# ShuhangGu/DASR

Measured on AMD Instinct MI355X. Metric: SR train images/sec (4x, 128->512), higher is better.
Workload: dtype bf16 MFMA operands, fp32 accumulate / fp32 residual stream

## Files before the change

dasr_amd/csrc/common.h:

```cpp
#pragma once
#include <hip/hip_runtime.h>
#include <hip/hip_ext.h>
#include <stdint.h>
#include "../../include/dasr_hip.h"

typedef __bf16 bf16_t;
typedef __attribute__((ext_vector_type(8))) __bf16 bf16x8;
typedef __attribute__((ext_vector_type(4))) __bf16 bf16x4;
typedef __attribute__((ext_vector_type(4))) short s16x4;
typedef _Float16 f16_t;
typedef __attribute__((ext_vector_type(8))) _Float16 f16x8;
typedef __attribute__((ext_vector_type(4))) _Float16 f16x4;
typedef __attribute__((ext_vector_type(16))) float f32x16;
typedef __attribute__((ext_vector_type(4))) float f32x4;
typedef __attribute__((ext_vector_type(4))) unsigned int u32x4;
typedef __attribute__((ext_vector_type(2))) unsigned int u32x2;

#define DASR_LDS __attribute__((address_space(3)))

#define HIP_TRY(expr)                                   \
    do {                                                \
        hipError_t _e = (expr);                         \
        if (_e != hipSuccess) return (int)_e;           \
    } while (0)

__device__ __forceinline__ float bf16_to_f32(bf16_t v) { return (float)v; }

__device__ __forceinline__ bf16_t f32_to_bf16(float v) { return (bf16_t)v; }

__device__ __forceinline__ void split_bf16(float v, bf16_t& hi, bf16_t& lo) {
    hi = (bf16_t)v;
    lo = (bf16_t)(v - (float)hi);
}

__device__ __forceinline__ void split_f16(float v, bf16_t& hi, bf16_t& lo) {
    const f16_t h = (f16_t)v;
    hi = __builtin_bit_cast(bf16_t, h);
    lo = __builtin_bit_cast(bf16_t, (f16_t)(v - (float)h));
}

template <bool F16>
__device__ __forceinline__ f32x16 mfma16(bf16x8 a, bf16x8 b, f32x16 c) {
    if constexpr (F16) return __builtin_amdgcn_mfma_f32_32x32x16_f16(__builtin_bit_cast(f16x8, a), __builtin_bit_cast(f16x8, b), c, 0, 0, 0);
    else return __builtin_amdgcn_mfma_f32_32x32x16_bf16(a, b, c, 0, 0, 0);
}

__device__ __forceinline__ float wave_sum(float v) {
#pragma unroll
    for (int o = 32; o > 0; o >>= 1) v += __shfl_xor(v, o, 64);
    return v;
}

static inline hipStream_t as_stream(void* s) { return (hipStream_t)s; }

struct dasr_red {
    float* part;
    unsigned* ticket;
};
dasr_red dasr_red_scratch(const void* key_acc, hipStream_t s, unsigned nblocks, int k);
int dasr_red_error();

template <int K>
__device__ __forceinline__ void grid_sum_commit(const dasr_red r, const float (&v)[K], float* const (&acc)[K], const float (&coef)[K]) {
    if (!r.part) return;
    __shared__ unsigned gs_last;
    __shared__ float gs_red[K][4];
    const unsigned nb = gridDim.x;
    if (threadIdx.x == 0) {
#pragma unroll
        for (int k = 0; k < K; ++k) __hip_atomic_store(r.part + (size_t)k * nb + blockIdx.x, v[k], __ATOMIC_RELAXED, __HIP_MEMORY_SCOPE_AGENT);
        asm volatile("s_waitcnt vmcnt(0)" ::: "memory");
        gs_last = __hip_atomic_fetch_add(r.ticket, 1u, __ATOMIC_RELAXED, __HIP_MEMORY_SCOPE_AGENT) == nb - 1u;
    }
    __syncthreads();
    if (!gs_last) return;
#pragma unroll
    for (int k = 0; k < K; ++k) {
        float s = 0.f;
        for (unsigned i = threadIdx.x; i < nb; i += 256u) s += __hip_atomic_load(r.part + (size_t)k * nb + i, __ATOMIC_RELAXED, __HIP_MEMORY_SCOPE_AGENT);
        s = wave_sum(s);
        if ((threadIdx.x & 63) == 0) gs_red[k][threadIdx.x >> 6] = s;
    }
    __syncthreads();
    if (threadIdx.x == 0) {
#pragma unroll
        for (int k = 0; k < K; ++k)
            if (acc[k]) atomicAdd(acc[k], ((gs_red[k][0] + gs_red[k][1]) + (gs_red[k][2] + gs_red[k][3])) * coef[k]);
        __hip_atomic_store(r.ticket, 0u, __ATOMIC_RELAXED, __HIP_MEMORY_SCOPE_AGENT);
    }
}

bool dasr_prof_slot(const char* tag, hipEvent_t* e0, hipEvent_t* e1);
#define DASR_LAUNCH_TAG(tag, kfn, grid, block, lds, s, ...)                                         \
    do {                                                                                            \
        hipEvent_t _e0 = nullptr, _e1 = nullptr;                                                    \
        if (dasr_prof_slot(tag, &_e0, &_e1)) hipExtLaunchKernelGGL(kfn, grid, block, lds, s, _e0, _e1, 0, __VA_ARGS__); \
        else hipLaunchKernelGGL(kfn, grid, block, lds, s, __VA_ARGS__);                             \
    } while (0)
#define DASR_LAUNCH(kfn, ...) DASR_LAUNCH_TAG(#kfn, kfn, __VA_ARGS__)
```

dasr_amd/csrc/misc.hip:

```cpp
#include "common.h"
#include <string.h>
#include <atomic>
#include <condition_variable>
#include <map>
#include <mutex>
#include <thread>
#include <tuple>

namespace {

__global__ void pack_kernel(const dasr_pack_desc* __restrict__ descs, int ndesc, long long total,
                            const long long* __restrict__ prefix, const float* __restrict__ params, bf16_t* __restrict__ packed) {
    const long long gid = (long long)blockIdx.x * blockDim.x + threadIdx.x;
    if (gid >= total) return;
    int lo = 0, hi = ndesc - 1;
    while (lo < hi) {
        const int mid = (lo + hi + 1) >> 1;
        if (prefix[mid] <= gid) lo = mid; else hi = mid - 1;
    }
    const dasr_pack_desc& D = descs[lo];
    long long q = gid - prefix[lo];
    const int lane = q & 63;
    q >>= 6;
    const int mi = q % D.mt;
    q /= D.mt;
    const int tap = q % D.ntaps;
    q /= D.ntaps;
    const int nchunks = D.cin_pad >> 4;
    const int ckv = q % nchunks;
    const int mg = q / nchunks;
    const int oc = (mg * D.mt + mi) * 32 + (lane & 31);
    const int kreal = D.fmt >= 3 ? nchunks / 3 : nchunks;
    const int part = ckv / kreal, ck = ckv - part * kreal;
    const int c0 = ck * 16 + 8 * (lane >> 5);
    bf16x8 vh, vl;
#pragma unroll
    for (int e = 0; e < 8; ++e) {
        const int cin = c0 + e;
        float v = 0.f;
        if (oc < D.cout) {
            for (int s = 0; s < D.nseg; ++s) {
                const dasr_pack_seg& S = D.seg[s];
                const int ci = cin - S.cin_start;
                if (ci >= 0 && ci < S.cin_len) {
                    const int st = D.tapmap[tap];
                    const unsigned msk = tap < 16 ? D.tapmask[tap] : 0u;
                    const bool okc = !S.transpose || ci < S.src_cout;
                    const long long base = !S.transpose ? S.src_off + ((long long)oc * S.src_cin + S.src_c0 + ci) * D.src_ntaps
                                                        : S.src_off + ((long long)ci * S.src_cin + S.src_c0 + oc) * D.src_ntaps;
                    if (msk && okc) {
                        float acc = 0.f;
                        for (int k = 0; k < D.src_ntaps && k < 16; ++k)
                            if (msk & (1u << k)) acc += params[base + k];
                        v = acc;
                    } else if (st >= 0 && okc) {
                        v = params[base + st];
                    }
                }
            }
        }
        bf16_t h, l;
        split_bf16(v, h, l);
        if (D.fmt == 1) h = __builtin_bit_cast(bf16_t, (f16_t)v);
        if (D.fmt == 2 || D.fmt == 3) split_f16(v, h, l);
        if (D.fmt >= 3 && part == 2) h = l;
        vh[e] = h;
        vl[e] = l;
    }
    const long long o = D.dst_off + (gid - prefix[lo]) * 8;
    *(bf16x8*)(packed + o) = vh;
    if (D.lo_off) *(bf16x8*)(packed + o + D.lo_off) = vl;
}

__global__ void nchw_to_blocked_kernel(const float* __restrict__ src, int N, int C, int H, int W, dasr_tensor df, dasr_tensor db) {
    const int ncb = (C + 15) >> 4;
    const long long total = (long long)N * ncb * H * W;
    const long long i = (long long)blockIdx.x * blockDim.x + threadIdx.x;
    if (i >= total) return;
    const int x = i % W;
    long long t = i / W;
    const int y = t % H;
    t /= H;
    const int cb = t % ncb;
    const int n = t / ncb;
    float v[16];
#pragma unroll
    for (int j = 0; j < 16; ++j) {
        const int c = cb * 16 + j;
        v[j] = c < C ? src[(((long long)n * C + c) * H + y) * W + x] : 0.f;
    }
    const size_t po = ((size_t)y * W + x) * 16;
    if (df.p) {
        float* d = (float*)df.p + (size_t)n * df.n_stride + (size_t)cb * df.cb_stride + po;
#pragma unroll
        for (int j = 0; j < 4; ++j) ((f32x4*)d)[j] = f32x4{v[4 * j], v[4 * j + 1], v[4 * j + 2], v[4 * j + 3]};
    }
    if (db.p) {
        bf16_t* d = (bf16_t*)db.p + (size_t)n * db.n_stride + (size_t)cb * db.cb_stride + po;
        bf16x8 a, b;
#pragma unroll
        for (int j = 0; j < 8; ++j) {
            a[j] = (bf16_t)v[j];
            b[j] = (bf16_t)v[8 + j];
        }
        ((bf16x8*)d)[0] = a;
        ((bf16x8*)d)[1] = b;
    }
}

__global__ void blocked_to_nchw_kernel(dasr_tensor s, int N, int C, int H, int W, float* __restrict__ dst) {
    const long long total = (long long)N * C * H * W;
    const long long i = (long long)blockIdx.x * blockDim.x + threadIdx.x;
    if (i >= total) return;
    const int x = i % W;
    long long t = i / W;
    const int y = t % H;
    t /= H;
    const int c = t % C;
    const int n = t / C;
    dst[i] = ((const float*)s.p)[(size_t)n * s.n_stride + (size_t)(c >> 4) * s.cb_stride + ((size_t)y * W + x) * 16 + (c & 15)];
}

__global__ void l1_loss_kernel(dasr_tensor sr, const float* __restrict__ hr, const float* __restrict__ wm, int N, int C, int H, int W,
                               float coef, float* loss_acc, dasr_tensor grad, int accumulate, float gscale, dasr_red rs) {
    const long long total = (long long)N * H * W;
    const long long i = (long long)blockIdx.x * blockDim.x + threadIdx.x;
    float part = 0.f;
    if (i < total) {
        const int x = i % W;
        long long t = i / W;
        const int y = t % H;
        const int n = t / H;
        const size_t po = ((size_t)y * W + x) * 16;
        const float* s = (const float*)sr.p + (size_t)n * sr.n_stride + po;
        const float wgt = wm ? wm[((long long)n * H + y) * W + x] : 1.f;
        float g[16];
#pragma unroll
        for (int j = 0; j < 16; ++j) g[j] = 0.f;
        for (int c = 0; c < C; ++c) {
            const float d = s[c] - hr[(((long long)n * C + c) * H + y) * W + x];
            if (accumulate & 2) {
                part += wgt * d * d;
                g[c] = 2.f * coef * wgt * d;
            } else {
                part += wgt * fabsf(d);
                g[c] = coef * wgt * (d > 0.f ? 1.f : (d < 0.f ? -1.f : 0.f));
            }
        }
        if (grad.p && (accumulate & 4)) {
            f16_t* gp = (f16_t*)grad.p + (size_t)n * grad.n_stride + po;
            for (int j = 0; j < (C + 3) / 4; ++j) {
                f16x4 o;
#pragma unroll
                for (int e = 0; e < 4; ++e) o[e] = (f16_t)(g[4 * j + e] * gscale);
                ((f16x4*)gp)[j] = o;
            }
        } else if (grad.p) {
            float* gp = (float*)grad.p + (size_t)n * grad.n_stride + po;
#pragma unroll
            for (int j = 0; j < 4; ++j) {
                f32x4 o = {g[4 * j], g[4 * j + 1], g[4 * j + 2], g[4 * j + 3]};
                if (accumulate & 1) o += ((const f32x4*)gp)[j];
                ((f32x4*)gp)[j] = o;
            }
        }
    }
    part = wave_sum(part);
    __shared__ float red[4];
    if ((threadIdx.x & 63) == 0) red[threadIdx.x >> 6] = part;
    __syncthreads();
    const float v[1] = {red[0] + red[1] + red[2] + red[3]};
    float* const acc[1] = {loss_acc};
    const float cf[1] = {coef};
    grid_sum_commit<1>(rs, v, acc, cf);
}

__global__ void downsum2x_kernel(dasr_tensor src, int N, int C, int H, int W, dasr_tensor mask, int mask_f32, float slope,
                                 dasr_tensor df, dasr_tensor db) {
    const int ncb = (C + 15) >> 4;
    const long long total = (long long)N * ncb * H * W * 4;
    const long long gi = (long long)blockIdx.x * blockDim.x + threadIdx.x;
    if (gi >= total) return;
    const int q = gi & 3;
    const long long i = gi >> 2;
    const int x = i % W;
    long long t = i / W;
    const int y = t % H;
    t /= H;
    const int cb = t % ncb;
    const int n = t / ncb;
    const float* s = (const float*)src.p + (size_t)n * src.n_stride + (size_t)cb * src.cb_stride + q * 4;
    const int W2 = 2 * W;
    f32x4 a = *(const f32x4*)(s + ((size_t)(2 * y) * W2 + 2 * x) * 16);
    a += *(const f32x4*)(s + ((size_t)(2 * y) * W2 + 2 * x + 1) * 16);
    a += *(const f32x4*)(s + ((size_t)(2 * y + 1) * W2 + 2 * x) * 16);
    a += *(const f32x4*)(s + ((size_t)(2 * y + 1) * W2 + 2 * x + 1) * 16);
    const size_t po = ((size_t)y * W + x) * 16 + q * 4;
    if (mask.p) {
        const size_t mo = (size_t)n * mask.n_stride + (size_t)cb * mask.cb_stride + po;
        float m[4];
        if (mask_f32) {
            const f32x4 mv = *(const f32x4*)((const float*)mask.p + mo);
            for (int j = 0; j < 4; ++j) m[j] = mv[j];
        } else {
            const bf16x4 mv = *(const bf16x4*)((const bf16_t*)mask.p + mo);
            for (int j = 0; j < 4; ++j) m[j] = (float)mv[j];
        }
        for (int j = 0; j < 4; ++j) a[j] = m[j] > 0.f ? a[j] : a[j] * slope;
    }
    if (df.p) *(f32x4*)((float*)df.p + (size_t)n * df.n_stride + (size_t)cb * df.cb_stride + po) = a;
    if (db.p) {
        bf16x4 o;
        for (int j = 0; j < 4; ++j) o[j] = (bf16_t)a[j];
        *(bf16x4*)((bf16_t*)db.p + (size_t)n * db.n_stride + (size_t)cb * db.cb_stride + po) = o;
    }
}

__global__ void axpby_kernel(dasr_tensor x, float a, dasr_tensor z, float b, int N, int C, int H, int W, dasr_tensor of,
                             dasr_tensor ob, float gamma, dasr_tensor mask, float slope, const float* slope_ptr) {
    const int ncb = (C + 15) >> 4;
    const long long per_plane = (long long)H * W * 4;
    const long long total = (long long)N * ncb * per_plane;
    const long long gi = (long long)blockIdx.x * blockDim.x + threadIdx.x;
    if (gi >= total) return;
    const long long e = (gi % per_plane) * 4;
    long long t = gi / per_plane;
    const int cb = t % ncb;
    const int n = t / ncb;
    f32x4 v = *(const f32x4*)((const float*)x.p + (size_t)n * x.n_stride + (size_t)cb * x.cb_stride + e) * a;
    if (z.p) v += *(const f32x4*)((const float*)z.p + (size_t)n * z.n_stride + (size_t)cb * z.cb_stride + e) * b;
    if (mask.p) {
        const float sl = slope_ptr ? *slope_ptr : slope;
        const f32x4 mv = *(const f32x4*)((const float*)mask.p + (size_t)n * mask.n_stride + (size_t)cb * mask.cb_stride + e);
        for (int j = 0; j < 4; ++j) v[j] = mv[j] > 0.f ? v[j] : v[j] * sl;
    }
    if (of.p) *(f32x4*)((float*)of.p + (size_t)n * of.n_stride + (size_t)cb * of.cb_stride + e) = v;
    if (ob.p) {
        bf16x4 o;
        for (int j = 0; j < 4; ++j) o[j] = (bf16_t)(v[j] * gamma);
        *(bf16x4*)((bf16_t*)ob.p + (size_t)n * ob.n_stride + (size_t)cb * ob.cb_stride + e) = o;
    }
}

__global__ void adam_kernel(float* __restrict__ p, const float* __restrict__ g, float* __restrict__ m, float* __restrict__ v,
                            long long n, float step_size, float beta1, float beta2, float eps, float wd, float inv_sqrt_bc2, int* __restrict__ nonfinite,
                            const int* __restrict__ gate) {
    if (gate && *gate != 0) return;
    bool bad = false;
    for (long long i = (long long)blockIdx.x * blockDim.x + threadIdx.x; i < n; i += (long long)gridDim.x * blockDim.x) {
        float gi = g[i];
        bad |= !(fabsf(gi) <= 3.0e38f);
        const float pi = p[i];
        if (wd != 0.f) gi += wd * pi;
        const float mi = beta1 * m[i] + (1.f - beta1) * gi;
        const float vi = beta2 * v[i] + (1.f - beta2) * gi * gi;
        m[i] = mi;
        v[i] = vi;
        const float denom = sqrtf(vi) * inv_sqrt_bc2 + eps;
        p[i] = pi - step_size * (mi / denom);
    }
    if (nonfinite && __any(bad) && (threadIdx.x & 63) == 0) atomicOr(nonfinite, 1);
}

__global__ void add_flat_kernel(float* __restrict__ y, const float* __restrict__ x, long long n) {
    for (long long i = (long long)blockIdx.x * blockDim.x + threadIdx.x; i < n; i += (long long)gridDim.x * blockDim.x) y[i] += x[i];
}

__global__ void fill_kernel(float* p, long long n, float v) {
    for (long long i = (long long)blockIdx.x * blockDim.x + threadIdx.x; i < n; i += (long long)gridDim.x * blockDim.x) p[i] = v;
}

inline unsigned blocks_for(long long total, int bs = 256) { return (unsigned)((total + bs - 1) / bs); }

}

extern "C" int dasr_pack_weights(const dasr_pack_desc* descs_dev, int32_t ndesc, int64_t total_pieces, const int64_t* piece_prefix_dev,
                                 const float* params_flat, void* packed, void* stream) {
    if (ndesc <= 0 || total_pieces <= 0) return DASR_EINVAL;
    DASR_LAUNCH(pack_kernel, dim3(blocks_for(total_pieces)), dim3(256), 0, as_stream(stream), descs_dev, ndesc,
                       (long long)total_pieces, (const long long*)piece_prefix_dev, params_flat, (bf16_t*)packed);
    return (int)hipGetLastError();
}

extern "C" int dasr_nchw_to_blocked(const float* src, int32_t N, int32_t C, int32_t H, int32_t W, dasr_tensor dst_f32,
                                    dasr_tensor dst_bf16, void* stream) {
    const long long total = (long long)N * ((C + 15) / 16) * H * W;
    if (total <= 0) return DASR_EINVAL;
    DASR_LAUNCH(nchw_to_blocked_kernel, dim3(blocks_for(total)), dim3(256), 0, as_stream(stream), src, N, C, H, W, dst_f32, dst_bf16);
    return (int)hipGetLastError();
}

extern "C" int dasr_blocked_to_nchw(dasr_tensor src, int32_t N, int32_t C, int32_t H, int32_t W, float* dst, void* stream) {
    const long long total = (long long)N * C * H * W;
    if (total <= 0) return DASR_EINVAL;
    DASR_LAUNCH(blocked_to_nchw_kernel, dim3(blocks_for(total)), dim3(256), 0, as_stream(stream), src, N, C, H, W, dst);
    return (int)hipGetLastError();
}

extern "C" int dasr_l1_loss(dasr_tensor sr, const float* hr_nchw, const float* weight_map, int32_t N, int32_t C, int32_t H, int32_t W,
                            float coef, float* loss_acc, dasr_tensor grad, int32_t accumulate, float grad_scale, void* stream) {
    const long long total = (long long)N * H * W;
    if (total <= 0 || C > 16) return DASR_EINVAL;
    if ((accumulate & 4) && (accumulate & 1)) return DASR_EINVAL;
    const dasr_red rs = dasr_red_scratch(loss_acc, as_stream(stream), blocks_for(total), 1);
    if (loss_acc && !rs.part) return dasr_red_error();
    DASR_LAUNCH(l1_loss_kernel, dim3(blocks_for(total)), dim3(256), 0, as_stream(stream), sr, hr_nchw, weight_map, N, C, H, W, coef,
                       loss_acc, grad, accumulate, grad_scale != 0.f ? grad_scale : 1.f, rs);
    return (int)hipGetLastError();
}

extern "C" int dasr_downsum2x(dasr_tensor src, int32_t N, int32_t C, int32_t H, int32_t W, dasr_tensor mask, int32_t mask_f32,
                              float slope, dasr_tensor dst_f32, dasr_tensor dst_bf16, void* stream) {
    const long long total = (long long)N * ((C + 15) / 16) * H * W * 4;
    if (total <= 0) return DASR_EINVAL;
    DASR_LAUNCH(downsum2x_kernel, dim3(blocks_for(total)), dim3(256), 0, as_stream(stream), src, N, C, H, W, mask, mask_f32, slope,
                       dst_f32, dst_bf16);
    return (int)hipGetLastError();
}

__device__ __forceinline__ float f32_rounded(float v) {
    asm("" : "+v"(v));
    return v;
}

__global__ void cvt_f16_kernel(dasr_tensor x, int N, int C, int H, int W, float scale, dasr_tensor y) {
    const int ncb = (C + 15) >> 4;
    const long long per_plane = (long long)H * W * 4, total = (long long)N * ncb * per_plane;
    const long long gi = (long long)blockIdx.x * blockDim.x + threadIdx.x;
    if (gi >= total) return;
    const long long e = (gi % per_plane) * 4;
    long long t = gi / per_plane;
    const int cb = t % ncb, n = t / ncb;
    const f32x4 v = *(const f32x4*)((const float*)x.p + (size_t)n * x.n_stride + (size_t)cb * x.cb_stride + e);
    f16x4 o;
    for (int j = 0; j < 4; ++j) o[j] = (f16_t)f32_rounded(v[j] * scale);
    *(f16x4*)((f16_t*)y.p + (size_t)n * y.n_stride + (size_t)cb * y.cb_stride + e) = o;
}

__global__ void f16_residual_kernel(dasr_tensor x, int N, int C, int H, int W, float scale, dasr_tensor y) {
    const int ncb = (C + 15) >> 4;
    const long long per_plane = (long long)H * W * 4, total = (long long)N * ncb * per_plane;
    const long long gi = (long long)blockIdx.x * blockDim.x + threadIdx.x;
    if (gi >= total) return;
    const long long e = (gi % per_plane) * 4;
    long long t = gi / per_plane;
    const int cb = t % ncb, n = t / ncb;
    const f32x4 v = *(const f32x4*)((const float*)x.p + (size_t)n * x.n_stride + (size_t)cb * x.cb_stride + e);
    const float inv = 1.f / scale;
    f32x4 o;
    for (int j = 0; j < 4; ++j) o[j] = v[j] - (float)(f16_t)f32_rounded(v[j] * scale) * inv;
    *(f32x4*)((float*)y.p + (size_t)n * y.n_stride + (size_t)cb * y.cb_stride + e) = o;
}

template <typename T>
__global__ void cvt_split16_kernel(dasr_tensor x, int N, int C, int H, int W, float scale, dasr_tensor y) {
    const int ncb = (C + 15) >> 4;
    const long long per_plane = (long long)H * W * 4, total = (long long)N * ncb * per_plane;
    const long long gi = (long long)blockIdx.x * blockDim.x + threadIdx.x;
    if (gi >= total) return;
    const long long e = (gi % per_plane) * 4;
    long long t = gi / per_plane;
    const int cb = t % ncb, n = t / ncb;
    const f32x4 v = *(const f32x4*)((const float*)x.p + (size_t)n * x.n_stride + (size_t)cb * x.cb_stride + e);
    T* yp = (T*)y.p + (size_t)n * y.n_stride + (size_t)cb * y.cb_stride + e;
    const size_t lo = (size_t)ncb * y.cb_stride;
#pragma unroll
    for (int j = 0; j < 4; ++j) {
        const float vv = f32_rounded(v[j] * scale);
        const T h = (T)vv;
        yp[j] = h;
        yp[lo + j] = (T)(vv - (float)h);
    }
}

__global__ void downsum2x_f16_kernel(dasr_tensor src, int N, int C, int H, int W, dasr_tensor mask, float slope, float out_scale, dasr_tensor df,
                                     dasr_tensor dh) {
    const int ncb = (C + 15) >> 4;
    const long long total = (long long)N * ncb * H * W * 4;
    const long long gi = (long long)blockIdx.x * blockDim.x + threadIdx.x;
    if (gi >= total) return;
    const int q = gi & 3;
    const long long i = gi >> 2;
    const int x = i % W;
    long long t = i / W;
    const int y = t % H;
    t /= H;
    const int cb = t % ncb, n = t / ncb;
    const f16_t* s = (const f16_t*)src.p + (size_t)n * src.n_stride + (size_t)cb * src.cb_stride + q * 4;
    const int W2 = 2 * W;
    float a[4] = {0.f, 0.f, 0.f, 0.f};
    for (int dy = 0; dy < 2; ++dy)
        for (int dx = 0; dx < 2; ++dx) {
            const f16x4 v = *(const f16x4*)(s + ((size_t)(2 * y + dy) * W2 + 2 * x + dx) * 16);
            for (int j = 0; j < 4; ++j) a[j] += (float)v[j];
        }
    const size_t po = ((size_t)y * W + x) * 16 + q * 4;
    if (mask.p) {
        const f16x4 mv = *(const f16x4*)((const f16_t*)mask.p + (size_t)n * mask.n_stride + (size_t)cb * mask.cb_stride + po);
        for (int j = 0; j < 4; ++j) a[j] = (float)mv[j] > 0.f ? a[j] : a[j] * slope;
    }
    for (int j = 0; j < 4; ++j) a[j] *= out_scale;
    if (df.p) *(f32x4*)((float*)df.p + (size_t)n * df.n_stride + (size_t)cb * df.cb_stride + po) = f32x4{a[0], a[1], a[2], a[3]};
    if (dh.p) {
        f16x4 o;
        for (int j = 0; j < 4; ++j) o[j] = (f16_t)a[j];
        *(f16x4*)((f16_t*)dh.p + (size_t)n * dh.n_stride + (size_t)cb * dh.cb_stride + po) = o;
    }
}

__global__ void pixel_shuffle_f16_kernel(dasr_tensor src, int N, int C4, int H, int W, dasr_tensor dst) {
    const int ncb = C4 >> 4;
    const long long total = (long long)N * ncb * H * W;
    const long long i = (long long)blockIdx.x * blockDim.x + threadIdx.x;
    if (i >= total) return;
    const int x = i % W;
    long long t = i / W;
    const int y = t % H;
    t /= H;
    const int p = t % ncb, n = t / ncb;
    const f16_t* s = (const f16_t*)src.p + (size_t)n * src.n_stride + (size_t)p * src.cb_stride + ((size_t)y * W + x) * 16;
    const f16x8 lo = *(const f16x8*)s, hi = *(const f16x8*)(s + 8);
    f16_t v[16];
    for (int j = 0; j < 8; ++j) { v[j] = lo[j]; v[8 + j] = hi[j]; }
    f16_t* d = (f16_t*)dst.p + (size_t)n * dst.n_stride + (size_t)(p >> 2) * dst.cb_stride + 4 * (p & 3);
    const int W2 = 2 * W;
    for (int k = 0; k < 4; ++k) {
        const f16x4 o = {v[k], v[4 + k], v[8 + k], v[12 + k]};
        *(f16x4*)(d + ((size_t)(2 * y + (k >> 1)) * W2 + 2 * x + (k & 1)) * 16) = o;
    }
}

__global__ void pixel_unshuffle_f16_kernel(dasr_tensor gsrc, dasr_tensor mask, float slope, int N, int C4, int H, int W, dasr_tensor gdst) {
    const int ncb = C4 >> 4;
    const long long total = (long long)N * ncb * H * W;
    const long long i = (long long)blockIdx.x * blockDim.x + threadIdx.x;
    if (i >= total) return;
    const int x = i % W;
    long long t = i / W;
    const int y = t % H;
    t /= H;
    const int p = t % ncb, n = t / ncb;
    const f16_t* g = (const f16_t*)gsrc.p + (size_t)n * gsrc.n_stride + (size_t)(p >> 2) * gsrc.cb_stride + 4 * (p & 3);
    const int W2 = 2 * W;
    f16_t v[16];
    for (int k = 0; k < 4; ++k) {
        const f16x4 q = *(const f16x4*)(g + ((size_t)(2 * y + (k >> 1)) * W2 + 2 * x + (k & 1)) * 16);
        for (int cc = 0; cc < 4; ++cc) v[4 * cc + k] = q[cc];
    }
    const size_t po = (size_t)n * gdst.n_stride + (size_t)p * gdst.cb_stride + ((size_t)y * W + x) * 16;
    if (mask.p) {
        const f16_t* m = (const f16_t*)mask.p + (size_t)n * mask.n_stride + (size_t)p * mask.cb_stride + ((size_t)y * W + x) * 16;
        for (int j = 0; j < 16; ++j) v[j] = (float)m[j] > 0.f ? v[j] : (f16_t)((float)v[j] * slope);
    }
    f16x8 lo, hi;
    for (int j = 0; j < 8; ++j) { lo[j] = v[j]; hi[j] = v[8 + j]; }
    *(f16x8*)((f16_t*)gdst.p + po) = lo;
    *(f16x8*)((f16_t*)gdst.p + po + 8) = hi;
}

extern "C" int dasr_pixel_shuffle_f16(dasr_tensor src, int32_t N, int32_t C4, int32_t H, int32_t W, dasr_tensor dst, void* stream) {
// ... 474 lines not shown
```

dasr_amd/csrc/wgrad.hip:

```cpp
#include "common.h"
#include <type_traits>

namespace {

template <int KH, int STRIDE>
struct WCfg {
    static constexpr int NTAPS = KH * KH;
    static constexpr int TAPS_PER_PART = NTAPS <= 16 ? NTAPS : 10;
    static constexpr int TPG = (TAPS_PER_PART + 1) / 2;
    static constexpr int PH = STRIDE == 2 ? 2 : ((KH == 3 || KH == 1) ? 8 : 4), PW = 16;
    static constexpr int IH = (PH - 1) * STRIDE + KH;
    static constexpr int IW = (PW - 1) * STRIDE + KH;
    static constexpr int GPLANE = PH * PW * 32 + 128;
    static constexpr int IPLANE_RAW = IH * IW * 32;
    static constexpr int IPLANE = IPLANE_RAW + ((IPLANE_RAW % 256) == 128 ? 0 : ((128 - (IPLANE_RAW % 256) + 256) % 256));
    static constexpr int G_BYTES = 2 * GPLANE;
    static constexpr int I_BYTES = 4 * IPLANE;
    static constexpr int LDS_BYTES = G_BYTES + I_BYTES;
};

template <bool F16>
__device__ __forceinline__ float frag_f32(bf16x8 a, int j) {
    if constexpr (F16) return (float)__builtin_bit_cast(f16x8, a)[j];
    else return (float)a[j];
// ... 447 lines not shown
        return;
    }
    const int pair = wave % 6, th = wave / 6;
    const int ot = pair >> 1, ct = pair & 1;
    const int n_ot = (P.g_planes + 1) >> 1;
    const bool active = ct < P.n_ctiles && ot < n_ot;
    f32x16 acc[5];
#pragma unroll
    for (int t = 0; t < 5; ++t)
#pragma unroll
        for (int j = 0; j < 16; ++j) acc[t][j] = 0.f;
    float bsum = 0.f;
    const int gg = lane >> 4, li = lane & 15;
    const int fplane = gg & 1, khalf = gg >> 1;
    const int gbase = (ot * 2 + fplane) * C::GPLANE + (8 * khalf + (li >> 2)) * 32 + (li & 3) * 8;
    const int ibase = C::G_BYTES + (ct * 2 + fplane) * C::IPLANE + (8 * khalf + (li >> 2)) * 32 + (li & 3) * 8;
    const bool want_bias = P.want_bias && ct == 0 && th == 0;
    __syncthreads();
    int cur = 0;
    auto run = [&](auto th_c) {
        constexpr int TH = decltype(th_c)::value;
        W3Win w;
        if (active) w3_win_prologue<TH>(smem, gbase, ibase, w);
        for (int tile = split; tile < ntiles; tile += nsplit) {
            const char* buf = smem + cur * C::BUF_BYTES;
            cur = cur == 2 ? 0 : cur + 1;
            if (active) w3_win_steps<F16, TH>(buf, gbase, ibase, w, acc, bsum, want_bias);
            __syncthreads();
            if (active) w3_win_last<F16, TH>(smem + cur * C::BUF_BYTES, gbase, ibase, w, acc, bsum, want_bias);
        }
    };
    if (th == 0) run(std::integral_constant<int, 0>{});
    else run(std::integral_constant<int, 1>{});
    if (active) {
        float* w = ws + P.ws_off + (size_t)split * 9 * 3 * 2048 + (size_t)ot * 2048;
        const int cin = ct * 32 + (lane & 31), h = lane >> 5;
        const int na = th ? 4 : 5;
#pragma unroll
        for (int t = 0; t < 5; ++t) {
            if (t < na) {
                const int tap = th ? (t == 0 ? 2 : t == 1 ? 5 : t == 2 ? 8 : 7) : (t == 0 ? 0 : t == 1 ? 3 : t == 2 ? 6 : t == 3 ? 1 : 4);
#pragma unroll
                for (int j = 0; j < 16; ++j) {
                    const int oc = (j & 3) + 8 * (j >> 2) + 4 * h;
                    w[(size_t)tap * 3 * 2048 + oc * 64 + cin] = acc[t][j];
                }
            }
        }
        if (want_bias) {
            const float tot = bsum + __shfl_xor(bsum, 32, 64);
            if (lane < 32) ws[P.ws_bias_off + (size_t)split * 96 + ot * 32 + lane] = tot;
        }
    }
}

template <bool F16>
__global__ __launch_bounds__(1024, 1) void wgrad3_ld_kernel(const dasr_wgrad_part* __restrict__ parts, int nparts, int nsplit_flags, float* __restrict__ ws) {
    wgrad3_ld_body<F16>(parts, nparts, nsplit_flags, ws);
}
__global__ __launch_bounds__(256) void wgrad_reduce_kernel(const dasr_wgrad_reduce_part* __restrict__ parts, int nparts,
                                                           const float* __restrict__ ws, float* __restrict__ grad, float scale) {
    __shared__ float red[16 * 16 * 17];
    const dasr_wgrad_reduce_part P = parts[blockIdx.y];
    const bool per_oc = gridDim.x == 32;
    const int oc = per_oc ? blockIdx.x : blockIdx.x >> 2, cg = per_oc ? 0 : blockIdx.x & 3, goc = P.oc0 + oc;
    if (goc >= P.cout) return;
    const int per = P.ntaps * 32 * 64;
    const long long sstride = P.split_stride > 0 ? P.split_stride : per, tstride = P.tap_stride > 0 ? P.tap_stride : 2048;
    const long long bstride = P.bias_stride > 0 ? P.bias_stride : 32;
    const int NT = P.ntaps_total > 0 ? P.ntaps_total : P.ntaps;
    const int ntaps = min(P.ntaps, NT - P.tap0);
    const int n_c = min(min(32 * P.n_ctiles, P.cin - P.c0), 64) - cg * 16;
    const int cl = threadIdx.x & 15, sl = threadIdx.x >> 4;
    if (P.nsplit <= 4 && ntaps <= 16) {
        if (cg != 0) return;
        const int n_all = min(min(32 * P.n_ctiles, P.cin - P.c0), 64);
        const int cgi = sl >> 2, sp = sl & 3, c = cgi * 16 + cl;
        if (c < n_all && sp < P.nsplit) {
            const float* src = ws + P.ws_off + (size_t)sp * sstride + oc * 64 + c;
            float q[16];
#pragma unroll
            for (int t = 0; t < 16; ++t) q[t] = t < ntaps ? src[(long long)t * tstride] : 0.f;
#pragma unroll
            for (int t = 0; t < 16; ++t)
                if (t < ntaps) red[(sl * 16 + cl) * 17 + t] = q[t];
        } else if (c < n_all) {
            for (int t = 0; t < ntaps; ++t) red[(sl * 16 + cl) * 17 + t] = 0.f;
        }
        __syncthreads();
        float* dst = grad + P.dst_w_off + ((long long)goc * P.cin + P.c0) * NT + P.tap0;
        const int nvalid = n_all * ntaps;
        for (int o = threadIdx.x; o < nvalid; o += 256) {
            const int cc = o / ntaps, tap = o - cc * ntaps;
            const float* r = red + (((cc >> 4) * 4) * 16 + (cc & 15)) * 17 + tap;
            const float tot = (r[0] + r[16 * 17]) + (r[2 * 16 * 17] + r[3 * 16 * 17]);
            dst[ntaps == NT ? (long long)o : (long long)cc * NT + tap] = tot * scale;
        }
        if (P.dst_b_off >= 0 && threadIdx.x < 64) {
            float b = threadIdx.x < (P.bias_nsplit > 0 ? P.bias_nsplit : P.nsplit) ? ws[P.ws_bias_off + (size_t)threadIdx.x * bstride + oc] : 0.f;
#pragma unroll
            for (int o = 32; o > 0; o >>= 1) b += __shfl_xor(b, o, 64);
            if (threadIdx.x == 0) grad[P.dst_b_off + goc] = b * scale;
        }
        return;
    }
    if (n_c > 0) {
        const float* src = ws + P.ws_off + oc * 64 + cg * 16 + cl;
        for (int tap0 = 0; tap0 < ntaps; tap0 += 3) {
            float a[3] = {0.f, 0.f, 0.f};
            if (cl < n_c) {
                for (int sp = sl; sp < P.nsplit; sp += 16 * 8) {
                    float q[3][8];
#pragma unroll
                    for (int t = 0; t < 3; ++t)
#pragma unroll
                        for (int k = 0; k < 8; ++k)
                            q[t][k] = (tap0 + t < ntaps && sp + 16 * k < P.nsplit) ? src[(size_t)(sp + 16 * k) * sstride + (long long)(tap0 + t) * tstride] : 0.f;
#pragma unroll
                    for (int t = 0; t < 3; ++t)
#pragma unroll
                        for (int k = 0; k < 8; ++k) a[t] += q[t][k];
                }
            }
#pragma unroll
            for (int t = 0; t < 3; ++t)
                if (tap0 + t < ntaps) red[(sl * 16 + cl) * 17 + tap0 + t] = a[t];
        }
    }
    __syncthreads();
    if (n_c > 0) {
        float* dst = grad + P.dst_w_off + ((long long)goc * P.cin + P.c0 + cg * 16) * NT + P.tap0;
        const int nvalid = (n_c < 16 ? n_c : 16) * ntaps;
        for (int o = threadIdx.x; o < nvalid; o += 256) {
            const int c = o / ntaps, tap = o - c * ntaps;
            const float* r = red + c * 17 + tap;
            float q[16];
#pragma unroll
            for (int k = 0; k < 16; ++k) q[k] = r[k * 16 * 17];
            const float tot = (((q[0] + q[1]) + (q[2] + q[3])) + ((q[4] + q[5]) + (q[6] + q[7]))) +
                              (((q[8] + q[9]) + (q[10] + q[11])) + ((q[12] + q[13]) + (q[14] + q[15])));
            dst[ntaps == NT ? (long long)o : (long long)c * NT + tap] = tot * scale;
        }
    }
    if (cg == 0 && P.dst_b_off >= 0 && threadIdx.x < 64) {
        float b = 0.f;
        const int nb_ = P.bias_nsplit > 0 ? P.bias_nsplit : P.nsplit;
        for (int sp = threadIdx.x; sp < nb_; sp += 64) b += ws[P.ws_bias_off + (size_t)sp * bstride + oc];
#pragma unroll
        for (int o = 32; o > 0; o >>= 1) b += __shfl_xor(b, o, 64);
        if (threadIdx.x == 0) grad[P.dst_b_off + goc] = b * scale;
    }
}

__global__ void probe_tr16_kernel(int* result) {
    __shared__ __attribute__((aligned(16))) short lds[4 * 64];
    const int l = threadIdx.x;
    for (int i = l; i < 256; i += 64) lds[i] = (short)(1000 * (i >> 6) + (i & 63));
    __syncthreads();
    const int gg = l >> 4, li = l & 15;
    const s16x4 v = __builtin_amdgcn_ds_read_tr16_b64_v4i16((DASR_LDS s16x4*)((char*)lds + gg * 128 + (li >> 2) * 32 + (li & 3) * 8));
    int ok = 1;
    for (int j = 0; j < 4; ++j) ok &= (v[j] == (short)(1000 * gg + 16 * j + li));
    const unsigned long long m = __ballot(ok);
    if (l == 0) *result = (m == ~0ull) ? 1 : 0;
}

template <int KH, int STRIDE, bool USE_TR, bool F32, bool F16 = false>
int launch_wgrad(const dasr_wgrad_part* parts, int nparts, int nsplit, float* ws, hipStream_t s) {
    using C = WCfg<KH, STRIDE>;
    auto kfn = wgrad_kernel<KH, STRIDE, USE_TR, F32, F16>;
    static bool attr_set = false;
    if (!attr_set) {
        HIP_TRY(hipFuncSetAttribute((const void*)kfn, hipFuncAttributeMaxDynamicSharedMemorySize, C::LDS_BYTES + 16));
        attr_set = true;
    }
    DASR_LAUNCH_TAG(__PRETTY_FUNCTION__, kfn, dim3(nparts * nsplit), dim3(256), C::LDS_BYTES + 16, s, parts, nparts, nsplit, ws);
    return (int)hipGetLastError();
}

template <bool F16>
int launch_wgrad3_ld(const dasr_wgrad_part* parts, int nparts, int nsplit, float* ws, hipStream_t s) {
    auto kfn = wgrad3_ld_kernel<F16>;
    static bool attr_set = false;
    if (!attr_set) {
        HIP_TRY(hipFuncSetAttribute((const void*)kfn, hipFuncAttributeMaxDynamicSharedMemorySize, W3L::LDS_BYTES));
        attr_set = true;
    }
    DASR_LAUNCH_TAG(__PRETTY_FUNCTION__, kfn, dim3(nparts * (nsplit & 0xffff)), dim3(W3L::NT), W3L::LDS_BYTES, s, parts, nparts, nsplit, ws);
    return (int)hipGetLastError();
}

int g_use_tr = -1;

}

extern "C" int dasr_probe_tr16(void* stream) {
    int* d = nullptr;
    HIP_TRY(hipMalloc(&d, sizeof(int)));
    DASR_LAUNCH(probe_tr16_kernel, dim3(1), dim3(64), 0, as_stream(stream), d);
    int h = -1;
    hipError_t e = hipMemcpyAsync(&h, d, sizeof(int), hipMemcpyDeviceToHost, as_stream(stream));
    if (e == hipSuccess) e = hipStreamSynchronize(as_stream(stream));
    (void)hipFree(d);
    if (e != hipSuccess) return -(int)e;
    g_use_tr = h;
    return h;
}

extern "C" int dasr_wgrad_set_mode(int use_tr) {
    if (use_tr & ~1) return DASR_EINVAL;
    g_use_tr = use_tr & 1;
    return 0;
}

namespace {
template <int KH, int STRIDE>
int dispatch_wgrad(const dasr_wgrad_part* parts, int nparts, int nsplit, bool tr, int f32, float* ws, hipStream_t s) {
    if (f32 & 2) {
        if (tr) return launch_wgrad<KH, STRIDE, true, true, true>(parts, nparts, nsplit, ws, s);
        return launch_wgrad<KH, STRIDE, false, true, true>(parts, nparts, nsplit, ws, s);
    }
    if (tr) return f32 ? launch_wgrad<KH, STRIDE, true, true>(parts, nparts, nsplit, ws, s) : launch_wgrad<KH, STRIDE, true, false>(parts, nparts, nsplit, ws, s);
    return f32 ? launch_wgrad<KH, STRIDE, false, true>(parts, nparts, nsplit, ws, s) : launch_wgrad<KH, STRIDE, false, false>(parts, nparts, nsplit, ws, s);
}
}

extern "C" int dasr_wgrad(const dasr_wgrad_part* parts_dev, int32_t nparts, int32_t nsplit, int32_t kh, int32_t stride, int32_t f32,
                          float* ws, void* stream) {
    hipStream_t s = as_stream(stream);
    if (nparts <= 0 || nsplit <= 0) return DASR_EINVAL;
    if (kh != 33 && (nsplit >> 16)) return DASR_EINVAL;
    if (kh == 33) {
        const int ns = nsplit & 0xffff, ppu = (nsplit >> 16) & 0xff;
        if (ns <= 0 || (nsplit >> 24) || (ppu && ((nparts % ppu) || (((long long)(nparts / ppu) * ns) & 7)))) return DASR_EINVAL;
    }
    if (g_use_tr < 0) return DASR_EINVAL;
    const bool tr = g_use_tr == 1;
    if (kh == 33) {
        if (!tr || f32 == 1) return DASR_EINVAL;
        return f32 == 2 ? launch_wgrad3_ld<true>(parts_dev, nparts, nsplit, ws, s) : launch_wgrad3_ld<false>(parts_dev, nparts, nsplit, ws, s);
    }
    if (kh == 3 && stride == 1) return dispatch_wgrad<3, 1>(parts_dev, nparts, nsplit, tr, f32, ws, s);
    if (kh == 4 && stride == 1) return dispatch_wgrad<4, 1>(parts_dev, nparts, nsplit, tr, f32, ws, s);
    if (kh == 4 && stride == 2) return dispatch_wgrad<4, 2>(parts_dev, nparts, nsplit, tr, f32, ws, s);
    if (kh == 5 && stride == 1) return dispatch_wgrad<5, 1>(parts_dev, nparts, nsplit, tr, f32, ws, s);
    if (kh == 1 && stride == 1) return dispatch_wgrad<1, 1>(parts_dev, nparts, nsplit, tr, f32, ws, s);
    if (kh == 3 && stride == 2) return dispatch_wgrad<3, 2>(parts_dev, nparts, nsplit, tr, f32, ws, s);
    return DASR_EINVAL;
}

extern "C" int dasr_wgrad_reduce(const dasr_wgrad_reduce_part* parts_dev, int32_t nparts, const float* ws, float* grad_flat,
                                 float scale, int32_t few_splits, void* stream) {
    if (nparts <= 0) return DASR_EINVAL;
    DASR_LAUNCH(wgrad_reduce_kernel, dim3(few_splits ? 32 : 128, nparts), dim3(256), 0, as_stream(stream), parts_dev, nparts, ws, grad_flat, scale);
    return (int)hipGetLastError();
}
```

Baseline: 549.2.

## Tile weight packing via LDS, batch L1 loss per block, add few-split wgrad reduce

```diff
diff --git a/dasr_amd/csrc/common.h b/dasr_amd/csrc/common.h
--- a/dasr_amd/csrc/common.h
+++ b/dasr_amd/csrc/common.h
@@ -90,6 +90,31 @@
     }
 }
 
+template <int V>
+__device__ __forceinline__ void grid_sum_commit_runs(const dasr_red r, const float (&v)[V], unsigned nruns, float* acc, float coef) {
+    if (!r.part) return;
+    __shared__ unsigned gs_last;
+    __shared__ float gs_red[4];
+    if (threadIdx.x == 0) {
+#pragma unroll
+        for (int u = 0; u < V; ++u)
+            if (blockIdx.x * V + u < nruns) __hip_atomic_store(r.part + blockIdx.x * V + u, v[u], __ATOMIC_RELAXED, __HIP_MEMORY_SCOPE_AGENT);
+        asm volatile("s_waitcnt vmcnt(0)" ::: "memory");
+        gs_last = __hip_atomic_fetch_add(r.ticket, 1u, __ATOMIC_RELAXED, __HIP_MEMORY_SCOPE_AGENT) == gridDim.x - 1u;
+    }
+    __syncthreads();
+    if (!gs_last) return;
+    float s = 0.f;
+    for (unsigned i = threadIdx.x; i < nruns; i += 256u) s += __hip_atomic_load(r.part + i, __ATOMIC_RELAXED, __HIP_MEMORY_SCOPE_AGENT);
+    s = wave_sum(s);
+    if ((threadIdx.x & 63) == 0) gs_red[threadIdx.x >> 6] = s;
+    __syncthreads();
+    if (threadIdx.x == 0) {
+        if (acc) atomicAdd(acc, ((gs_red[0] + gs_red[1]) + (gs_red[2] + gs_red[3])) * coef);
+        __hip_atomic_store(r.ticket, 0u, __ATOMIC_RELAXED, __HIP_MEMORY_SCOPE_AGENT);
+    }
+}
+
 bool dasr_prof_slot(const char* tag, hipEvent_t* e0, hipEvent_t* e1);
 #define DASR_LAUNCH_TAG(tag, kfn, grid, block, lds, s, ...)                                         \
     do {                                                                                            \
diff --git a/dasr_amd/csrc/misc.hip b/dasr_amd/csrc/misc.hip
--- a/dasr_amd/csrc/misc.hip
+++ b/dasr_amd/csrc/misc.hip
@@ -9,17 +9,15 @@
 
 namespace {
 
-__global__ void pack_kernel(const dasr_pack_desc* __restrict__ descs, int ndesc, long long total,
-                            const long long* __restrict__ prefix, const float* __restrict__ params, bf16_t* __restrict__ packed) {
-    const long long gid = (long long)blockIdx.x * blockDim.x + threadIdx.x;
-    if (gid >= total) return;
-    int lo = 0, hi = ndesc - 1;
-    while (lo < hi) {
-        const int mid = (lo + hi + 1) >> 1;
-        if (prefix[mid] <= gid) lo = mid; else hi = mid - 1;
-    }
-    const dasr_pack_desc& D = descs[lo];
-    long long q = gid - prefix[lo];
+__device__ __forceinline__ void pack_round(int fmt, int part, float v, bf16_t& h, bf16_t& l) {
+    split_bf16(v, h, l);
+    if (fmt == 1) h = __builtin_bit_cast(bf16_t, (f16_t)v);
+    if (fmt == 2 || fmt == 3) split_f16(v, h, l);
+    if (fmt >= 3 && part == 2) h = l;
+}
+
+__device__ __forceinline__ void pack_piece(const dasr_pack_desc& D, long long piece, const float* __restrict__ params, bf16_t* __restrict__ packed) {
+    long long q = piece;
     const int lane = q & 63;
     q >>= 6;
     const int mi = q % D.mt;
@@ -60,16 +58,106 @@
             }
         }
         bf16_t h, l;
-        split_bf16(v, h, l);
-        if (D.fmt == 1) h = __builtin_bit_cast(bf16_t, (f16_t)v);
-        if (D.fmt == 2 || D.fmt == 3) split_f16(v, h, l);
-        if (D.fmt >= 3 && part == 2) h = l;
+        pack_round(D.fmt, part, v, h, l);
         vh[e] = h;
         vl[e] = l;
     }
-    const long long o = D.dst_off + (gid - prefix[lo]) * 8;
+    const long long o = D.dst_off + piece * 8;
     *(bf16x8*)(packed + o) = vh;
     if (D.lo_off) *(bf16x8*)(packed + o + D.lo_off) = vl;
+}
+
+constexpr int PACK_WG_PIECES = 1152;
+constexpr int PACK_LDS_FWD = 145;
+constexpr int PACK_LDS_TR = 577;
+
+__device__ __forceinline__ bool pack_desc_is_plain(const dasr_pack_desc& D) {
+    if (D.nseg != 1 || D.fmt > 2 || D.fmt < 0 || D.ntaps != 9 || D.src_ntaps != 9 || D.mt < 1 || D.mt > 2 || D.seg[0].cin_start != 0) return false;
+    unsigned m = 0;
+#pragma unroll
+    for (int t = 0; t < 9; ++t) m |= D.tapmask[t];
+    return m == 0;
+}
+
+__device__ __forceinline__ void pack_plain_rows(const dasr_pack_desc& D, long long row0, long long row1, const float* __restrict__ params,
+                                                bf16_t* __restrict__ packed, float* tile) {
+    const dasr_pack_seg& S = D.seg[0];
+    const int rpt = 9 * D.mt, nchunks = D.cin_pad >> 4, noc = 32 * D.mt;
+    const bool tr = S.transpose != 0;
+    const int nrun = tr ? 16 : noc, runlen = tr ? noc * 9 : 144, rstride = tr ? PACK_LDS_TR : PACK_LDS_FWD;
+    const int wave = threadIdx.x >> 6, lane = threadIdx.x & 63;
+    for (long long t = row0 / rpt; t * rpt < row1; ++t) {
+        const int mg = (int)(t / nchunks), ck = (int)(t - (long long)mg * nchunks);
+        const int oc0 = mg * noc, ci0 = ck * 16;
+        const int ci_end = tr ? min(S.cin_len, S.src_cout) : S.cin_len;
+        const int nci = max(0, min(16, ci_end - ci0)), nocv = max(0, min(noc, D.cout - oc0));
+        const int vrun = tr ? nci : nocv, vlen = tr ? nocv * 9 : nci * 9;
+        const long long base0 = tr ? S.src_off + ((long long)ci0 * S.src_cin + S.src_c0 + oc0) * 9 : S.src_off + ((long long)oc0 * S.src_cin + S.src_c0 + ci0) * 9;
+        const long long rowstep = (long long)S.src_cin * 9;
+        const bool vec = ((base0 | rowstep) & 3) == 0 && ((uintptr_t)params & 15) == 0;
+        __syncthreads();
+        const int nv4 = runlen >> 2;
+        for (int i = threadIdx.x; i < nrun * nv4; i += 256) {
+            const int r = i / nv4, k = (i - r * nv4) * 4;
+            const float* src = params + base0 + r * rowstep + k;
+            f32x4 v = {0.f, 0.f, 0.f, 0.f};
+            if (r < vrun) {
+                if (vec && k + 4 <= vlen) {
+                    v = *(const f32x4*)src;
+                } else {
+#pragma unroll
+                    for (int e = 0; e < 4; ++e)
+                        if (k + e < vlen) v[e] = src[e];
+                }
+            }
+            float* d = tile + r * rstride + k;
+#pragma unroll
+            for (int e = 0; e < 4; ++e) d[e] = v[e];
+        }
+        __syncthreads();
+        const long long ra = max(row0, t * rpt), rb = min(row1, (t + 1) * rpt);
+        for (long long row = ra + wave; row < rb; row += 4) {
+            const int rr = (int)(row - t * rpt), tap = rr / D.mt, mi = rr - tap * D.mt;
+            const int st = D.tapmap[tap];
+            const int ocl = mi * 32 + (lane & 31), j0 = 8 * (lane >> 5);
+            bf16x8 vh, vl;
+#pragma unroll
+            for (int e = 0; e < 8; ++e) {
+                const float v = st >= 0 ? (tr ? tile[(j0 + e) * PACK_LDS_TR + ocl * 9 + st] : tile[ocl * PACK_LDS_FWD + (j0 + e) * 9 + st]) : 0.f;
+                bf16_t h, l;
+                pack_round(D.fmt, 0, v, h, l);
+                vh[e] = h;
+                vl[e] = l;
+            }
+            const long long o = D.dst_off + (row * 64 + lane) * 8;
+            *(bf16x8*)(packed + o) = vh;
+            if (D.lo_off) *(bf16x8*)(packed + o + D.lo_off) = vl;
+        }
+    }
+}
+
+__global__ __launch_bounds__(256) void pack_kernel(const dasr_pack_desc* __restrict__ descs, int ndesc, long long total,
+                                                   const long long* __restrict__ prefix, const float* __restrict__ params, bf16_t* __restrict__ packed) {
+    __shared__ float tile[64 * PACK_LDS_FWD];
+    long long g0 = (long long)blockIdx.x * PACK_WG_PIECES;
+    const long long g1 = min(g0 + PACK_WG_PIECES, total);
+    if (g0 >= g1) return;
+    int lo = 0, hi = ndesc - 1;
+    while (lo < hi) {
+        const int mid = (lo + hi + 1) >> 1;
+        if (prefix[mid] <= g0) lo = mid; else hi = mid - 1;
+    }
+    for (int d = lo; d < ndesc && g0 < g1; ++d) {
+        const long long p0 = prefix[d], e = min(g1, prefix[d + 1]);
+        if (e <= g0) continue;
+        const dasr_pack_desc& D = descs[d];
+        if (pack_desc_is_plain(D)) {
+            pack_plain_rows(D, (g0 - p0) >> 6, (e - p0) >> 6, params, packed, tile);
+        } else {
+            for (long long q = g0 - p0 + threadIdx.x; q < e - p0; q += 256) pack_piece(D, q, params, packed);
+        }
+        g0 = e;
+    }
 }
 
 __global__ void nchw_to_blocked_kernel(const float* __restrict__ src, int N, int C, int H, int W, dasr_tensor df, dasr_tensor db) {
@@ -121,58 +209,79 @@
     dst[i] = ((const float*)s.p)[(size_t)n * s.n_stride + (size_t)(c >> 4) * s.cb_stride + ((size_t)y * W + x) * 16 + (c & 15)];
 }
 
-__global__ void l1_loss_kernel(dasr_tensor sr, const float* __restrict__ hr, const float* __restrict__ wm, int N, int C, int H, int W,
-                               float coef, float* loss_acc, dasr_tensor grad, int accumulate, float gscale, dasr_red rs) {
+constexpr int L1_RUNS = 4;
+template <int CC>
+__global__ __launch_bounds__(256) void l1_loss_kernel(dasr_tensor sr, const float* __restrict__ hr, const float* __restrict__ wm, int N, int C_, int H, int W,
+                                                      float coef, float* loss_acc, dasr_tensor grad, int accumulate, float gscale, dasr_red rs) {
+    const int C = CC ? CC : C_;
     const long long total = (long long)N * H * W;
-    const long long i = (long long)blockIdx.x * blockDim.x + threadIdx.x;
-    float part = 0.f;
-    if (i < total) {
-        const int x = i % W;
-        long long t = i / W;
-        const int y = t % H;
-        const int n = t / H;
-        const size_t po = ((size_t)y * W + x) * 16;
-        const float* s = (const float*)sr.p + (size_t)n * sr.n_stride + po;
-        const float wgt = wm ? wm[((long long)n * H + y) * W + x] : 1.f;
-        float g[16];
-#pragma unroll
-        for (int j = 0; j < 16; ++j) g[j] = 0.f;
-        for (int c = 0; c < C; ++c) {
-            const float d = s[c] - hr[(((long long)n * C + c) * H + y) * W + x];
-            if (accumulate & 2) {
-                part += wgt * d * d;
-                g[c] = 2.f * coef * wgt * d;
-            } else {
-                part += wgt * fabsf(d);
-                g[c] = coef * wgt * (d > 0.f ? 1.f : (d < 0.f ? -1.f : 0.f));
+    float part[L1_RUNS];
+#pragma unroll
+    for (int u = 0; u < L1_RUNS; ++u) {
+        const long long i = ((long long)blockIdx.x * L1_RUNS + u) * 256 + threadIdx.x;
+        part[u] = 0.f;
+        if (i < total) {
+            const int x = i % W;
+            long long t = i / W;
+            const int y = t % H;
+            const int n = t / H;
+            const size_t po = ((size_t)y * W + x) * 16;
+            const float* s = (const float*)sr.p + (size_t)n * sr.n_stride + po;
+            const float wgt = wm ? wm[((long long)n * H + y) * W + x] : 1.f;
+            float sv[16], g[16];
+            if (CC && CC <= 4) {
+                const f32x4 q = *(const f32x4*)s;
+#pragma unroll
+                for (int j = 0; j < 4; ++j) sv[j] = q[j];
             }
-        }
-        if (grad.p && (accumulate & 4)) {
-            f16_t* gp = (f16_t*)grad.p + (size_t)n * grad.n_stride + po;
-            for (int j = 0; j < (C + 3) / 4; ++j) {
-                f16x4 o;
-#pragma unroll
-                for (int e = 0; e < 4; ++e) o[e] = (f16_t)(g[4 * j + e] * gscale);
-                ((f16x4*)gp)[j] = o;
+#pragma unroll
+            for (int j = 0; j < 16; ++j) g[j] = 0.f;
+#pragma unroll
+            for (int c = 0; c < (CC ? CC : 16); ++c) {
+                if (c < C) {
+                    const float d = ((CC && CC <= 4) ? sv[c] : s[c]) - hr[(((long long)n * C + c) * H + y) * W + x];
+                    if (accumulate & 2) {
+                        part[u] += wgt * d * d;
+                        g[c] = 2.f * coef * wgt * d;
+                    } else {
+                        part[u] += wgt * fabsf(d);
+                        g[c] = coef * wgt * (d > 0.f ? 1.f : (d < 0.f ? -1.f : 0.f));
+                    }
+                }
             }
-        } else if (grad.p) {
-            float* gp = (float*)grad.p + (size_t)n * grad.n_stride + po;
-#pragma unroll
-            for (int j = 0; j < 4; ++j) {
-                f32x4 o = {g[4 * j], g[4 * j + 1], g[4 * j + 2], g[4 * j + 3]};
-                if (accumulate & 1) o += ((const f32x4*)gp)[j];
-                ((f32x4*)gp)[j] = o;
+            if (grad.p && (accumulate & 4)) {
+                f16_t* gp = (f16_t*)grad.p + (size_t)n * grad.n_stride + po;
+#pragma unroll
+                for (int j = 0; j < 4; ++j) {
+                    if (j < (C + 3) / 4) {
+                        f16x4 o;
+#pragma unroll
+                        for (int e = 0; e < 4; ++e) o[e] = (f16_t)(g[4 * j + e] * gscale);
+                        ((f16x4*)gp)[j] = o;
+                    }
+                }
+            } else if (grad.p) {
+                float* gp = (float*)grad.p + (size_t)n * grad.n_stride + po;
+#pragma unroll
+                for (int j = 0; j < 4; ++j) {
+                    f32x4 o = {g[4 * j], g[4 * j + 1], g[4 * j + 2], g[4 * j + 3]};
+                    if (accumulate & 1) o += ((const f32x4*)gp)[j];
+                    ((f32x4*)gp)[j] = o;
+                }
             }
         }
     }
-    part = wave_sum(part);
-    __shared__ float red[4];
-    if ((threadIdx.x & 63) == 0) red[threadIdx.x >> 6] = part;
+    __shared__ float red[L1_RUNS][4];
+#pragma unroll
+    for (int u = 0; u < L1_RUNS; ++u) {
+        const float p = wave_sum(part[u]);
+        if ((threadIdx.x & 63) == 0) red[u][threadIdx.x >> 6] = p;
+    }
     __syncthreads();
-    const float v[1] = {red[0] + red[1] + red[2] + red[3]};
-    float* const acc[1] = {loss_acc};
-    const float cf[1] = {coef};
-    grid_sum_commit<1>(rs, v, acc, cf);
+    float v[L1_RUNS];
+#pragma unroll
+    for (int u = 0; u < L1_RUNS; ++u) v[u] = red[u][0] + red[u][1] + red[u][2] + red[u][3];
+    grid_sum_commit_runs<L1_RUNS>(rs, v, (unsigned)((total + 255) / 256), loss_acc, coef);
 }
 
 __global__ void downsum2x_kernel(dasr_tensor src, int N, int C, int H, int W, dasr_tensor mask, int mask_f32, float slope,
@@ -277,7 +386,7 @@
 extern "C" int dasr_pack_weights(const dasr_pack_desc* descs_dev, int32_t ndesc, int64_t total_pieces, const int64_t* piece_prefix_dev,
                                  const float* params_flat, void* packed, void* stream) {
     if (ndesc <= 0 || total_pieces <= 0) return DASR_EINVAL;
-    DASR_LAUNCH(pack_kernel, dim3(blocks_for(total_pieces)), dim3(256), 0, as_stream(stream), descs_dev, ndesc,
+    DASR_LAUNCH(pack_kernel, dim3(blocks_for(total_pieces, PACK_WG_PIECES)), dim3(256), 0, as_stream(stream), descs_dev, ndesc,
                        (long long)total_pieces, (const long long*)piece_prefix_dev, params_flat, (bf16_t*)packed);
     return (int)hipGetLastError();
 }
@@ -304,8 +413,13 @@
     if ((accumulate & 4) && (accumulate & 1)) return DASR_EINVAL;
     const dasr_red rs = dasr_red_scratch(loss_acc, as_stream(stream), blocks_for(total), 1);
     if (loss_acc && !rs.part) return dasr_red_error();
-    DASR_LAUNCH(l1_loss_kernel, dim3(blocks_for(total)), dim3(256), 0, as_stream(stream), sr, hr_nchw, weight_map, N, C, H, W, coef,
-                       loss_acc, grad, accumulate, grad_scale != 0.f ? grad_scale : 1.f, rs);
+    const dim3 grid(blocks_for(total, 256 * L1_RUNS));
+    if (C == 3)
+        DASR_LAUNCH(l1_loss_kernel<3>, grid, dim3(256), 0, as_stream(stream), sr, hr_nchw, weight_map, N, C, H, W, coef, loss_acc, grad, accumulate,
+                    grad_scale != 0.f ? grad_scale : 1.f, rs);
+    else
+        DASR_LAUNCH(l1_loss_kernel<0>, grid, dim3(256), 0, as_stream(stream), sr, hr_nchw, weight_map, N, C, H, W, coef, loss_acc, grad, accumulate,
+                    grad_scale != 0.f ? grad_scale : 1.f, rs);
     return (int)hipGetLastError();
 }
 
diff --git a/dasr_amd/csrc/wgrad.hip b/dasr_amd/csrc/wgrad.hip
--- a/dasr_amd/csrc/wgrad.hip
+++ b/dasr_amd/csrc/wgrad.hip
@@ -623,6 +623,61 @@
     }
 }
 
+constexpr int RF_OCS = 64 * 16 + 1;
+__global__ __launch_bounds__(256) void wgrad_reduce_few_kernel(const dasr_wgrad_reduce_part* __restrict__ parts, int nparts,
+                                                               const float* __restrict__ ws, float* __restrict__ grad, float scale) {
+    __shared__ float red[4 * RF_OCS];
+    const dasr_wgrad_reduce_part P = parts[blockIdx.y];
+    const int wave = threadIdx.x >> 6, lane = threadIdx.x & 63;
+    const long long sstride = P.split_stride > 0 ? P.split_stride : (long long)P.ntaps * 32 * 64, tstride = P.tap_stride > 0 ? P.tap_stride : 2048;
+    const long long bstride = P.bias_stride > 0 ? P.bias_stride : 32;
+    const int NT = P.ntaps_total > 0 ? P.ntaps_total : P.ntaps;
+    const int ntaps = min(P.ntaps, NT - P.tap0);
+    const int n_all = min(min(32 * P.n_ctiles, P.cin - P.c0), 64);
+    {
+        const int ocl = lane >> 4, c4 = lane & 15, oc = blockIdx.x * 4 + ocl;
+        const bool vec = (((unsigned long long)P.ws_off | (unsigned long long)sstride | (unsigned long long)tstride) & 3) == 0 && ((uintptr_t)ws & 15) == 0;
+        const float* src = ws + P.ws_off + oc * 64 + c4 * 4;
+        if (P.oc0 + oc < P.cout && c4 * 4 < n_all) {
+            for (int t = wave; t < ntaps; t += 4) {
+                f32x4 q[4];
+#pragma unroll
+                for (int sp = 0; sp < 4; ++sp) {
+                    q[sp] = f32x4{0.f, 0.f, 0.f, 0.f};
+                    if (sp < P.nsplit) {
+                        const float* a = src + (size_t)sp * sstride + (long long)t * tstride;
+                        if (vec) q[sp] = *(const f32x4*)a;
+                        else q[sp] = f32x4{a[0], a[1], a[2], a[3]};
+                    }
+                }
+                const f32x4 tot = (q[0] + q[1]) + (q[2] + q[3]);
+#pragma unroll
+                for (int e = 0; e < 4; ++e) red[ocl * RF_OCS + (c4 * 4 + e) * ntaps + t] = tot[e];
+            }
+        }
+    }
+    __syncthreads();
+    const int oc = blockIdx.x * 4 + wave, goc = P.oc0 + oc;
+    if (goc >= P.cout) return;
+    float* dst = grad + P.dst_w_off + ((long long)goc * P.cin + P.c0) * NT + P.tap0;
+    const int nvalid = n_all * ntaps;
+    for (int o = lane; o < nvalid; o += 64) {
+        const float tot = red[wave * RF_OCS + o];
+        if (ntaps == NT) {
+            dst[o] = tot * scale;
+        } else {
+            const int cc = o / ntaps, tap = o - cc * ntaps;
+            dst[(long long)cc * NT + tap] = tot * scale;
+        }
+    }
+    if (P.dst_b_off >= 0) {
+        float b = lane < (P.bias_nsplit > 0 ? P.bias_nsplit : P.nsplit) ? ws[P.ws_bias_off + (size_t)lane * bstride + oc] : 0.f;
+#pragma unroll
+        for (int o = 32; o > 0; o >>= 1) b += __shfl_xor(b, o, 64);
+        if (lane == 0) grad[P.dst_b_off + goc] = b * scale;
+    }
+}
+
 __global__ void probe_tr16_kernel(int* result) {
     __shared__ __attribute__((aligned(16))) short lds[4 * 64];
     const int l = threadIdx.x;
@@ -723,6 +778,9 @@
 extern "C" int dasr_wgrad_reduce(const dasr_wgrad_reduce_part* parts_dev, int32_t nparts, const float* ws, float* grad_flat,
                                  float scale, int32_t few_splits, void* stream) {
     if (nparts <= 0) return DASR_EINVAL;
-    DASR_LAUNCH(wgrad_reduce_kernel, dim3(few_splits ? 32 : 128, nparts), dim3(256), 0, as_stream(stream), parts_dev, nparts, ws, grad_flat, scale);
+    if (few_splits)
+        DASR_LAUNCH(wgrad_reduce_few_kernel, dim3(8, nparts), dim3(256), 0, as_stream(stream), parts_dev, nparts, ws, grad_flat, scale);
+    else
+        DASR_LAUNCH(wgrad_reduce_kernel, dim3(128, nparts), dim3(256), 0, as_stream(stream), parts_dev, nparts, ws, grad_flat, scale);
     return (int)hipGetLastError();
 }
```

Measured after the change: 553.8 (median of 6 runs). No clear change (+0.8%).
